# arghyasur1991/Spark-TTS

Measured on AMD Instinct MI355X. Metric: audio samples/sec (whole node), Spark-TTS-0.5B greedy, higher is better.
Workload: dtype bf16 weights + KV, fp32 activations/accumulate (LLM); vocoder: fp32 operands split into 2 bf16 planes, 3 products on the bf16 matrix pipe, fp32 accumulate

## Files before the change

spark-tts_amd/csrc/smi_llm.hip:

```cpp
#include "smi_common.h"
#include <stdio.h>
#include <string.h>
#include <cmath>
#include <map>
#include <mutex>
#include <vector>

namespace {

constexpr int kMaxRows = SMI_MAX_ROWS;
constexpr int kHeadDim = 64;

struct RowDesc {
  int32_t slot, pos, token, flags;
};

struct SampRec {
  int32_t mode;
  int32_t top_k;
  float inv_temp, top_p;
  unsigned long long seed;
  int32_t has_seed, pad;
};

// ... 1853 lines not shown
constexpr int kFuseOT = 2;

__device__ __forceinline__ void attn_merge(const float* wmax, const float (*pw)[kHeadDim], const float* pl, int d,
                                           float& bm, float& O, float& Ls) {
  constexpr float LOG2E = 1.4426950408889634f;
  float wm[kAttnWaves], po[kAttnWaves], pls[kAttnWaves];
#pragma unroll
  for (int w = 0; w < kAttnWaves; ++w) { wm[w] = wmax[w]; po[w] = pw[w][d]; pls[w] = pl[w]; }
  bm = wm[0];
#pragma unroll
  for (int w = 1; w < kAttnWaves; ++w) bm = fmaxf(bm, wm[w]);
  O = 0.f; Ls = 0.f;
#pragma unroll
  for (int w = 0; w < kAttnWaves; ++w) {
    const float sc = exp2f((wm[w] - bm) * LOG2E);
    O += po[w] * sc; Ls += pls[w] * sc;
  }
}

__device__ __forceinline__ void attn_merge_split(const float* wmax, const float (*pw)[kHeadDim], const float* pl, int d,
                                                 uint32_t& hi, uint32_t& mi, uint32_t& lo) {
  float bm, O, Ls;
  attn_merge(wmax, pw, pl, d, bm, O, Ls);
  split3(O / Ls, hi, mi, lo);
}

__device__ __forceinline__ void attn_put_pieces(unsigned char* xs, int d, uint32_t hi, uint32_t mi, uint32_t lo) {
  unsigned char* q = xs + (size_t)((d >> 5) * 12 + ((d >> 3) & 3)) * 16 + (d & 7) * 2;
  *(uint16_t*)q = (uint16_t)hi;
  *(uint16_t*)(q + 64) = (uint16_t)mi;
  *(uint16_t*)(q + 128) = (uint16_t)lo;
}

template <int KVF32, int ONE = 0, int FUSE = 0, int PG = 0>
__global__ __launch_bounds__((FUSE ? 2 : 1) * kAttnWaves * 64) void k_attn(AttnP p) {
  static_assert(!FUSE || (FUSE == 1 && ONE == 1) || (FUSE == 2 && ONE == 2), "fused o_proj: one row (per-head partials for gate_up) or 2..8 rows (last-arriver head sum)");
  constexpr int LPT = KVF32 ? 16 : 8;
  constexpr int DPL = kHeadDim / LPT;
  constexpr int TPW = 64 / LPT;
  constexpr int NGRP = kAttnWaves * TPW;
  constexpr int UNR = 4;
  constexpr float NEG = -1e30f;
  constexpr float LOG2E = 1.4426950408889634f;
  __shared__ float wmax[kAttnWaves];
  __shared__ __attribute__((aligned(16))) float so[kAttnWaves][TPW][kHeadDim];
  __shared__ float sl[kAttnWaves][TPW];
  __shared__ float pw[kAttnWaves][kHeadDim], pl[kAttnWaves];
  __shared__ __attribute__((aligned(16))) unsigned char xsl[FUSE == 1 ? kAttnWaves * 2 * 3 * 4 * 16 : FUSE ? 2 * 3 * 4 * 16 : 16];
  __shared__ unsigned int s_last;
  const int tid = threadIdx.x, lane = tid & 63, wave = tid >> 6;
  if constexpr (ONE == 1) {
    if constexpr (FUSE) asm volatile("" ::"s"(p.q), "s"(p.work_blocks), "s"(p.Wo), "s"(gridDim.x));
    else asm volatile("" ::"s"(p.q), "s"(p.work_blocks), "s"(gridDim.x));
  }
  if ((int)blockIdx.x >= p.work_blocks) {
    pf_run(p.pf, (int)blockIdx.x - p.work_blocks, (int)gridDim.x - p.work_blocks, tid, (FUSE ? 2 : 1) * kAttnWaves * 64);
    return;
  }
  unsigned fbid = blockIdx.x;
  if constexpr (FUSE == 2) {
    const unsigned total = (unsigned)p.work_blocks, xcd = fbid & 7u, slot = fbid >> 3, q8 = total >> 3, r8 = total & 7u;
    fbid = xcd * q8 + (xcd < r8 ? xcd : r8) + slot;
  }
  const int f_head = FUSE ? (int)(fbid % (unsigned)p.n_heads) : 0, f_q = FUSE ? (int)(fbid / (unsigned)p.n_heads) % kFuseQB : 0,
            f_row = FUSE == 2 ? (int)(fbid / (unsigned)(p.n_heads * kFuseQB)) : 0;
  if constexpr (FUSE) {
    if (wave >= kAttnWaves) {
      const int fq = f_q, fper = p.NTo / kFuseQB, fh = f_head;
      const int ow = wave - kAttnWaves, KTo = 2 * p.n_heads;
// ... 41 lines not shown
          }
        }
      }
      if constexpr (FUSE != 2) return;
      else asm volatile("s_waitcnt vmcnt(0)" ::: "memory");
    }
  }
  if (!FUSE || wave < kAttnWaves) {
  unsigned bid = blockIdx.x;
  if (ONE != 1) {
    const unsigned total = (unsigned)p.work_blocks, xcd = bid & 7u, slot = bid >> 3, q8 = total >> 3, r8 = total & 7u;
    bid = xcd * q8 + (xcd < r8 ? xcd : r8) + slot;
  }
  const int head = FUSE == 2 ? f_head : ONE == 1 ? (FUSE ? (int)bid % p.n_heads : (int)bid) : ONE == 2 ? (int)bid % p.n_heads : (int)(bid / p.nseg) % p.n_heads,
            m = FUSE == 2 ? f_row : ONE == 1 ? 0 : ONE == 2 ? (int)bid / p.n_heads : (int)bid / (p.nseg * p.n_heads),
            seg = ONE ? 0 : (int)bid % p.nseg;
  const int tl = lane / LPT, dl = lane % LPT;
  const int grp = wave * TPW + tl;
  const RowDesc rd = p.rows[m];
  const int kvh = head / p.group;
  const bool sir = ONE || p.slot_is_row;
  const int slot = sir ? m : rd.slot;
  const size_t rowbase = ((size_t)slot * p.n_kv + kvh) * p.max_pos;
  const int ctx_all = rd.pos + 1;
  int ctx = ctx_all < (seg + 1) * kAttnSeg ? ctx_all : (seg + 1) * kAttnSeg;
  if (!ONE && seg * kAttnSeg >= ctx_all) return;

  float qraw[DPL];
  {
    const float* qp = p.q + (size_t)m * p.q_dim + head * kHeadDim + dl * DPL;
#pragma unroll
    for (int i = 0; i < DPL; ++i) qraw[i] = qp[i];
  }
  float m_run = NEG, lrun = 0.f, o[DPL];
#pragma unroll
  for (int i = 0; i < DPL; ++i) o[i] = 0.f;

  int c0 = seg * kAttnSeg;
  do {
    uint4 kr[UNR], vr[UNR];
#pragma unroll
    for (int u = 0; u < UNR; ++u) {
      const int t = c0 + u * NGRP + grp;
      const int tc = sir ? (t < p.max_pos ? t : p.max_pos - 1) : (t < ctx ? t : ctx - 1);
      const size_t off = ((ONE && !PG) ? rowbase + tc : kv_row(p.km, slot, kvh, p.n_kv, p.max_pos, tc)) * kHeadDim + dl * DPL;
      if (KVF32) {
        kr[u] = *(const uint4*)((const float*)p.kcache + off);
        vr[u] = *(const uint4*)((const float*)p.vcache + off);
      } else {
        kr[u] = *(const uint4*)((const uint16_t*)p.kcache + off);
        vr[u] = *(const uint4*)((const uint16_t*)p.vcache + off);
      }
    }
    if (ONE) {
      int pr = rd.pos;
      asm volatile("" : "+v"(pr));
      ctx = pr + 1 < kAttnSeg ? pr + 1 : kAttnSeg;
    }
    float qv[DPL];
#pragma unroll
    for (int i = 0; i < DPL; ++i) {
      float t = qraw[i];
      asm volatile("" : "+v"(t));
      qv[i] = t * 0.125f;
    }
    float sc[UNR];
    float lmax = NEG;
#pragma unroll
    for (int u = 0; u < UNR; ++u) {
      const uint32_t ku[4] = {kr[u].x, kr[u].y, kr[u].z, kr[u].w};
      float d = 0.f;
      if (KVF32) {
#pragma unroll
        for (int i = 0; i < 4; ++i) d += qv[i % DPL] * __uint_as_float(ku[i]);
      } else {
#pragma unroll
        for (int i = 0; i < 4; ++i) {
          d += qv[(2 * i) % DPL] * __uint_as_float(ku[i] << 16);
          d += qv[(2 * i + 1) % DPL] * __uint_as_float(ku[i] & 0xffff0000u);
        }
      }
      d = KVF32 ? smi_sum16(d) : smi_sum8(d);
      sc[u] = (c0 + u * NGRP + grp < ctx) ? d : NEG;
      lmax = fmaxf(lmax, sc[u]);
    }
    lmax = fmaxf(lmax, smi_dpp<0x128>(lmax));
    const float wm = fmaxf(fmaxf(smi_readlane(lmax, 0), smi_readlane(lmax, 16)), fmaxf(smi_readlane(lmax, 32), smi_readlane(lmax, 48)));
    const float mn = fmaxf(m_run, wm);
    const float a = exp2f((m_run - mn) * LOG2E);
    lrun *= a;
#pragma unroll
    for (int i = 0; i < DPL; ++i) o[i] *= a;
#pragma unroll
    for (int u = 0; u < UNR; ++u) {
      const float e = sc[u] > 0.5f * NEG ? exp2f((sc[u] - mn) * LOG2E) : 0.f;
      const uint32_t vu[4] = {vr[u].x, vr[u].y, vr[u].z, vr[u].w};
      lrun += e;
      if (KVF32) {
#pragma unroll
        for (int i = 0; i < 4; ++i) o[i % DPL] += e * __uint_as_float(vu[i]);
      } else {
#pragma unroll
        for (int i = 0; i < 4; ++i) {
          o[(2 * i) % DPL] += e * __uint_as_float(vu[i] << 16);
          o[(2 * i + 1) % DPL] += e * __uint_as_float(vu[i] & 0xffff0000u);
        }
      }
    }
    m_run = mn;
    c0 += NGRP * UNR;
  } while (c0 < ctx);
#pragma unroll
  for (int i = 0; i < DPL; i += 4)
    *(float4*)&so[wave][tl][dl * DPL + i] = make_float4(o[i], o[i + 1], o[i + 2], o[i + 3]);
  if (dl == 0) sl[wave][tl] = lrun;
  asm volatile("s_waitcnt lgkmcnt(0)" ::: "memory");
  {
    float O = 0.f, Ls = 0.f;
#pragma unroll
    for (int g = 0; g < TPW; ++g) { O += so[wave][g][lane]; Ls += sl[wave][g]; }
    pw[wave][lane] = O;
    if (lane == 0) { pl[wave] = Ls; wmax[wave] = m_run; }
  }
  __syncthreads();
  if constexpr (FUSE == 1) return;
  if (tid < kHeadDim) {
    if (!ONE && p.nseg > 1) {
      float bm, O, Ls;
      attn_merge(wmax, pw, pl, tid, bm, O, Ls);
      float* pp = p.part + (((size_t)m * p.n_heads + head) * p.nseg + seg) * 66;
      pp[2 + tid] = O;
      if (tid == 0) { pp[0] = bm; pp[1] = Ls; }
      return;
    }
    uint32_t hi, mi, lo;
    attn_merge_split(wmax, pw, pl, tid, hi, mi, lo);
    if constexpr (FUSE) {
      attn_put_pieces(xsl, tid, hi, mi, lo);
    } else {
      const int Mx = ONE == 1 ? 1 : p.M;
      const size_t ob = xs_off(o_ktile(head, tid, p.n_heads), 0, (tid >> 3) & 3, m, Mx) + (tid & 7) * 2;
      const size_t pl2 = (size_t)4 * Mx * 16;
      *(uint16_t*)(p.xs_out + ob) = (uint16_t)hi;
      *(uint16_t*)(p.xs_out + ob + pl2) = (uint16_t)mi;
// ... 1007 lines not shown
  int pg_split_rows;
  int pg_forced;
  float *part_o, *h2;
  float4* dpart;
  int dc_min;
  int fuse_o;
  int fuse1_last;
  int fuse2_rows;
  unsigned int* fuse_cnt;
  RowDesc* rows;
  RowDesc* plan;
  PfTile* pf_tiles;
  size_t pf_tiles_cap;
  int pf_ntiles;
  std::vector<PfTile> host_tiles;
  int attn_pf2;
  size_t plan_cap;
  float* pval; int* pidx; int lm_blocks, lm_cap;
  int64_t* hist; int32_t *count, *finished, *step;
  void *kcache, *vcache; size_t kv_layer_elems;
  int B; int started;
  int paged, pshift, ppslot;
  int32_t* ptab;
  std::vector<int32_t> hptab;
  std::vector<int32_t> free_pages;
  std::vector<int32_t> page_ref;
  int slot_pages[kMaxRows];
  int plen[kMaxRows];
  Ctl hctl; Ctl* ctl;
  int admit_seq;
  int session, identity_slots;
  std::vector<int> live_order;
  int attn_seg;
  float* apart; size_t apart_floats;
  int slot_busy[kMaxRows], slot_len[kMaxRows];
  int max_len, steps_launched;
  int do_sample, top_k; float temperature, top_p; unsigned long long seed;
  int slot_samp[kMaxRows];
  int slot_pen[kMaxRows];
  int slot_lp[kMaxRows];
  int slot_allow[kMaxRows];
  int lm_restrict;
  int* tlist;
  std::vector<int32_t> host_tlist;
  float* lp;
  float* lp_part; float2* lp_rowc;
  uint16_t* phist;
  int64_t* poll_dev; int64_t* poll_host;
  int32_t* pen_idx; size_t pen_idx_cap;
  std::vector<int32_t> host_pen_idx;
  float* logits; int* tok;
  float* cand_v; int* cand_i; unsigned int* cand_n;
  unsigned long long* stamps; int stamps_on;
  int max_steps;
  int tune[4];
  int graph_steps;
  int pf_inline;
  int pf_qkv_eighths;
  int prefetch_mask, prefetch_rows;
  int tune2;
  int pgemm_min_rows;
  int pg_min[4];
  int wd_parts;
  int exact;
  int gu1_lo;
  int gu1_rows;
  hipGraphExec_t graph; int graph_B, graph_seg, graph_ident, graph_samp, graph_pen, graph_lp, graph_allow;
  std::map<hipGraphExec_t, hipStream_t> graph_last;
  std::map<uint64_t, hipGraphExec_t> graph_cache;
  hipEvent_t ev0, ev1;
  std::vector<RowDesc> host_rows;
#ifdef SMI_DIAG
  EngState eng;
  int eng_on;
#endif
};

namespace {

std::vector<const void*>& lds_big_kernels() {
  static std::vector<const void*> v;
  return v;
}
bool lds_big_register(const void* f) {
  lds_big_kernels().push_back(f);
  return true;
}
template <auto F>
struct LdsBig {
  static inline const bool reg = lds_big_register((const void*)F);
};
constexpr int kLdsBigBytes = 160 * 1024;

void pages_release(smi_llm* L, int slot) {
  for (int i = 0; i < L->slot_pages[slot]; ++i) {
    const int32_t pg = L->hptab[(size_t)slot * L->ppslot + i];
    if (--L->page_ref[pg] == 0) L->free_pages.push_back(pg);
  }
  L->slot_pages[slot] = 0;
}
// ... 31 lines not shown
  return SMI_OK;
}
KvMap kv_map(const smi_llm* L) { return KvMap{L->paged ? L->ptab : nullptr, L->pshift, L->ppslot}; }
bool samp_any(const smi_llm* L) {
  if (L->do_sample) return true;
  for (int sl = 0; sl < kMaxRows; ++sl)
    if (L->slot_samp[sl]) return true;
  return false;
}
bool pen_any(const smi_llm* L) {
  for (int sl = 0; sl < kMaxRows; ++sl)
    if (L->slot_pen[sl]) return true;
  return false;
}
bool lp_any(const smi_llm* L) {
  for (int sl = 0; sl < kMaxRows; ++sl)
    if (L->slot_lp[sl]) return true;
  return false;
}
bool allow_any(const smi_llm* L) {
  for (int sl = 0; sl < kMaxRows; ++sl)
    if (L->slot_allow[sl]) return true;
  return false;
}
bool lm_restricted(const smi_llm* L) {
  return L->lm_restrict && L->KTh <= 32 && !L->exact && allow_any(L);
}
bool logits_needed(const smi_llm* L) {
  return samp_any(L) || pen_any(L) || lp_any(L) || (allow_any(L) && !lm_restricted(L));
}
int allow_bits(const smi_llm* L) { return allow_any(L) ? (lm_restricted(L) ? 3 : 1) : 0; }
uint64_t graph_key(const smi_llm* L, int samp, int pen, int lp, int K) {
  return (uint64_t)L->B | ((uint64_t)L->attn_seg << 8) | ((uint64_t)(L->identity_slots ? 1 : 0) << 24) | ((uint64_t)samp << 25) |
         ((uint64_t)pen << 26) | ((uint64_t)lp << 27) | ((uint64_t)allow_bits(L) << 28) | ((uint64_t)K << 32);
}
void graphs_flush(smi_llm* L) {
  std::vector<hipStream_t> drained;
  for (auto& gl : L->graph_last) {
    bool seen = false;
    for (hipStream_t d : drained) seen |= d == gl.second;
    if (!seen) { (void)hipStreamSynchronize(gl.second); drained.push_back(gl.second); }
  }
  L->graph_last.clear();
  for (auto& kv : L->graph_cache) if (kv.second) (void)hipGraphExecDestroy(kv.second);
  L->graph_cache.clear();
  L->graph = nullptr;
}

template <int MT, int NTB, int NW, int U, int WB, int PRO, int EPI, int H = 1, int OCC = 1>
int launch_gemm_kv(const smi_llm* L, GemmP p, hipStream_t st) {
  const int work = (p.NT + NTB - 1) / NTB * H;
  p.work_blocks = work;
  p.stamps = L->stamps_on ? L->stamps : nullptr;
  if constexpr (MT == 1 && NTB == 1 && NW == 16 && H == 4 && PRO == PRO_PLAIN && EPI == EPI_RESID) {
    if (p.M == 1 && !p.stamps && p.KT <= 160 && !(L->tune2 & 1048576)) {
      const int helpers = (L->prefetch_mask & 4) && p.pf.base && work < 232 ? ((L->tune2 & 4194304) ? 224 : (256 - work) / 8 * 8) : 0;
      if (p.KT <= 32) hipLaunchKernelGGL(k_down1<2>, dim3(work + helpers), dim3(256), 0, st, p);
      else if (p.KT <= 96) hipLaunchKernelGGL(k_down1<6>, dim3(work + helpers), dim3(256), 0, st, p);
      else hipLaunchKernelGGL(k_down1<10>, dim3(work + helpers), dim3(256), 0, st, p);
      SMI_LAUNCH_CHECK();
      return SMI_OK;
    }
    if (p.M >= 2 && p.M <= 8 && !p.stamps && p.KT <= 160 && !(L->tune2 & 2097152)) {
      const dim3 g(work), b(256);
      if (p.M <= 4) {
        if (p.KT <= 32) hipLaunchKernelGGL((k_downS<2, 1>), g, b, 0, st, p);
        else if (p.KT <= 96) hipLaunchKernelGGL((k_downS<6, 1>), g, b, 0, st, p);
// ... 222 lines not shown

enum { KQKV = 0, KATTN, KO, KGU, KD, KLM, KFIN };
enum { PF_GROUPED = 1, PF_PGEMM = 2 };
constexpr int kPgSplitRows = 512;
constexpr int kPgSegO = 2, kPgSegD = 8;

int ensure_apart(smi_llm* L, size_t floats) {
  if (floats <= L->apart_floats) return SMI_OK;
  graphs_flush(L);
  if (L->apart) (void)hipFree(L->apart);
  L->apart = nullptr; L->apart_floats = 0;
  if (hipMalloc((void**)&L->apart, floats * 4) != hipSuccess) { smi_set_error("hipMalloc(attention partials, %zu floats) failed", floats); return SMI_ENOMEM; }
  L->apart_floats = floats;
  return SMI_OK;
}

int lm_blocks_for(const smi_llm* L, int M) {
  if (L->KTh > 32 || L->exact) return L->lm_cap;
  return M <= 16 ? L->lm_blocks : (L->lm_blocks < 256 ? L->lm_blocks : 256);
}

int pen_set_ids(int V, int nblk) { return ((V + nblk - 1) / nblk + 3) & ~3; }

LpP lp_params(const smi_llm* L, int M) {
  LpP lp;
  lp.logits = L->logits; lp.ctl = L->ctl; lp.rows = L->rows; lp.pval = L->pval; lp.nblk = lm_blocks_for(L, M);
  lp.V = L->cfg.vocab_size; lp.per = pen_set_ids(lp.V, kLpBlocks); lp.inv_temp = 1.0f / L->temperature; lp.hs = L->do_sample;
  lp.part = L->lp_part; lp.rowc = L->lp_rowc;
  return lp;
}

int segs_for(int ctx_bound) { return ctx_bound <= kAttnSeg ? 1 : (ctx_bound + kAttnSeg - 1) / kAttnSeg; }

template <int KVF32>
int launch_attn(smi_llm* L, AttnP a, int helpers_ok, hipStream_t st) {
  a.nseg = L->attn_seg < 1 ? 1 : L->attn_seg;
  a.work_blocks = a.n_heads * a.M * a.nseg;
  const bool fuse = a.M == 1 && a.nseg == 1 && a.slot_is_row && a.part_o && !a.cnt;
  const bool fuse2 = a.nseg == 1 && a.slot_is_row && a.part_o && a.cnt;
  if (fuse || fuse2) a.work_blocks *= kFuseQB;
  if (a.nseg > 1) {
    int rc = ensure_apart(L, (size_t)a.M * a.n_heads * a.nseg * 66);
    if (rc) return rc;
    a.part = L->apart;
  }
  const int helpers = (helpers_ok && (L->prefetch_mask & 2) && a.M <= L->prefetch_rows && a.work_blocks < 232) ? (256 - a.work_blocks) / 8 * 8 : 0;
  const bool pg = a.km.ptab != nullptr;
#ifdef SMI_DIAG
  if (fuse2 && pg)
    hipLaunchKernelGGL((k_attn<KVF32, 2, 2, 1>), dim3(a.work_blocks), dim3(2 * kAttnWaves * 64), 0, st, a);
  else if (fuse2)
    hipLaunchKernelGGL((k_attn<KVF32, 2, 2>), dim3(a.work_blocks), dim3(2 * kAttnWaves * 64), 0, st, a);
  else
#endif
  if (fuse && pg)
    hipLaunchKernelGGL((k_attn<KVF32, 1, 1, 1>), dim3(a.work_blocks + helpers), dim3(2 * kAttnWaves * 64), 0, st, a);
  else if (fuse)
    hipLaunchKernelGGL((k_attn<KVF32, 1, 1>), dim3(a.work_blocks + helpers), dim3(2 * kAttnWaves * 64), 0, st, a);
  else if (a.M == 1 && a.nseg == 1 && a.slot_is_row && pg)
    hipLaunchKernelGGL((k_attn<KVF32, 1, 0, 1>), dim3(a.work_blocks + helpers), dim3(kAttnWaves * 64), 0, st, a);
  else if (a.M == 1 && a.nseg == 1 && a.slot_is_row)
    hipLaunchKernelGGL((k_attn<KVF32, 1>), dim3(a.work_blocks + helpers), dim3(kAttnWaves * 64), 0, st, a);
  else if (a.nseg == 1 && a.slot_is_row && pg)
    hipLaunchKernelGGL((k_attn<KVF32, 2, 0, 1>), dim3(a.work_blocks + helpers), dim3(kAttnWaves * 64), 0, st, a);
  else if (a.nseg == 1 && a.slot_is_row)
    hipLaunchKernelGGL((k_attn<KVF32, 2>), dim3(a.work_blocks + helpers), dim3(kAttnWaves * 64), 0, st, a);
  else
    hipLaunchKernelGGL((k_attn<KVF32, 0>), dim3(a.work_blocks + helpers), dim3(kAttnWaves * 64), 0, st, a);
  SMI_LAUNCH_CHECK();
  if (a.nseg > 1) {
    hipLaunchKernelGGL(k_attn_merge, dim3(a.M), dim3(1024), 0, st, a);
    SMI_LAUNCH_CHECK();
  }
  return SMI_OK;
}

bool fuse_o_now(const smi_llm* L, const RowDesc* rows, int M) {
  return L->fuse_o && !L->fuse1_last && M == 1 && rows == L->rows && L->identity_slots && L->attn_seg <= 1;
}
bool fuse2_now(const smi_llm* L, const RowDesc* rows, int M) {
  return L->fuse_o && M >= (L->fuse1_last ? 1 : 2) && M <= L->fuse2_rows && rows == L->rows && L->identity_slots && L->attn_seg <= 1;
}

int launch_oproj(const smi_llm* L, const GemmP& p, int M, hipStream_t st) {
  switch (L->cfg.num_heads) {
    case 14: return M <= 8 ? launch_gemm<1, 14, 2, 1, PRO_PLAIN, EPI_RESID, 4>(L, p, st) : launch_gemm<1, 14, 2, 1, PRO_PLAIN, EPI_RESID, 1, 0>(L, p, st);
    case 4: return M <= 8 ? launch_gemm<1, 4, 2, 1, PRO_PLAIN, EPI_RESID, 4>(L, p, st) : launch_gemm<1, 4, 2, 1, PRO_PLAIN, EPI_RESID, 1, 0>(L, p, st);
    default:
      return M <= 8 ? launch_gemm<1, 8, 4, 1, PRO_PLAIN, EPI_RESID, 4>(L, p, st) : launch_gemm<1, 8, 4, 1, PRO_PLAIN, EPI_RESID, 1, 0>(L, p, st);
  }
}

template <int TPC, int MTN>
int launch_down_chains_t(const smi_llm* L, const DownCP& d, hipStream_t st) {
  const size_t lds = (size_t)TPC * 12 * (d.M < MTN * 16 ? d.M : MTN * 16) * 16;
  static_cast<void>(LdsBig<k_downC<TPC, MTN>>::reg);
// ... 487 lines not shown
  { L->tune[0] = L->tune[1] = L->tune[2] = L->tune[3] = 0; const char* e = smi_env("SPARKMI_TUNE"); if (e) sscanf(e, "%d,%d,%d,%d", &L->tune[0], &L->tune[1], &L->tune[2], &L->tune[3]); }
  L->bh = L->bq = nullptr; L->bxs_h = L->bxs_attn = L->bxs_act = nullptr; L->bss = nullptr; L->big_rows = 0;
  L->pslab = nullptr; L->pslab_bytes = 0;
  L->prefetch_mask = 1; L->prefetch_rows = 1;
  if (const char* e = smi_env("SPARKMI_PREFETCH")) { L->prefetch_mask = atoi(e) & 7; L->prefetch_rows = 8; }
  if (smi_env("SPARKMI_NO_PREFETCH")) L->prefetch_mask = 0;
  { const char* e = smi_env("SPARKMI_GRAPH_STEPS"); L->graph_steps = e ? atoi(e) : 8; if (L->graph_steps < 1 || L->graph_steps > 32) L->graph_steps = 8; }
  { const char* e = smi_env("SPARKMI_PF_INLINE"); L->pf_inline = !(e && e[0] == '0'); }
  { const char* e = smi_env("SPARKMI_PF_QKV"); L->pf_qkv_eighths = e ? atoi(e) : 2; if (L->pf_qkv_eighths < 0 || L->pf_qkv_eighths > 8) L->pf_qkv_eighths = 2; }
  L->part_o = nullptr; L->h2 = nullptr; L->dpart = nullptr; L->fuse_cnt = nullptr;
  { const char* e = smi_env("SPARKMI_FUSE1_LAST"); L->fuse1_last = e && e[0] == '1'; }
  { const char* e = smi_env("SPARKMI_FUSE2_ROWS"); L->fuse2_rows = e ? atoi(e) : 0; if (L->fuse2_rows > kFuse2Max) L->fuse2_rows = kFuse2Max; }
  { const char* e = smi_env("SPARKMI_DC_MIN"); L->dc_min = e ? atoi(e) : 7; }
  L->fuse_o = !smi_env("SPARKMI_NO_FUSE_O") && (cfg->num_heads == 14 || cfg->num_heads == 4) && cfg->num_heads <= kMaxOHeads &&
              L->NTh % kFuseQB == 0 && L->NTh / kFuseQB <= kAttnWaves * kFuseOT && L->KTh * 8 <= 256;
  { const char* e = smi_env("SPARKMI_TUNE2"); L->tune2 = e ? atoi(e) : 0; }
  { const char* e = smi_env("SPARKMI_PGEMM_MIN_ROWS"); L->pgemm_min_rows = e ? atoi(e) : 1280; }
  {
    const char* names[4] = {"SPARKMI_PGEMM_MIN_QKV", "SPARKMI_PGEMM_MIN_O", "SPARKMI_PGEMM_MIN_GU", "SPARKMI_PGEMM_MIN_D"};
    const int dflt[4] = {1280, 1280, 288, 896};
    const bool common = smi_env("SPARKMI_PGEMM_MIN_ROWS") != nullptr;
    L->pg_forced = common;
    for (int i = 0; i < 4; ++i) { const char* e = smi_env(names[i]); L->pg_forced |= e != nullptr; L->pg_min[i] = e ? atoi(e) : common ? L->pgemm_min_rows : dflt[i]; }
  }
  { const char* e = smi_env("SPARKMI_PG_SPLIT_ROWS"); L->pg_split_rows = e ? atoi(e) : kPgSplitRows; if (L->pg_split_rows > kPgSplitRows) L->pg_split_rows = kPgSplitRows; }
  { const char* e = smi_env("SPARKMI_PF_LONG"); L->pf_long = e ? atoi(e) : kMaxRows + 1; if (L->pf_long < kMaxRows + 1) L->pf_long = kMaxRows + 1; }
  { const char* e = smi_env("SPARKMI_GU1_ROWS"); L->gu1_rows = e ? atoi(e) : 32; }
  { const char* e = smi_env("SPARKMI_GU1_LO"); L->gu1_lo = e ? atoi(e) : 4; }
  L->wd_parts = cfg->wd_plain ? 0 : 1;
  L->exact = cfg->weights_exact;
  if (L->exact) L->fuse_o = 0;
  L->pf_tiles = nullptr; L->pf_tiles_cap = 0; L->pf_ntiles = 0;
  { const char* e = smi_env("SPARKMI_ATTN_PF2"); L->attn_pf2 = !(e && e[0] == '0'); }
  L->graph = nullptr; L->graph_B = 0; L->graph_seg = 1; L->graph_ident = 1; L->graph_samp = 0; L->graph_pen = 0; L->graph_lp = 0; L->graph_allow = 0; memset(L->slot_samp, 0, sizeof(L->slot_samp)); memset(L->slot_pen, 0, sizeof(L->slot_pen));
  memset(L->slot_lp, 0, sizeof(L->slot_lp)); L->lp = nullptr; L->lp_part = nullptr; L->lp_rowc = nullptr;
  memset(L->slot_allow, 0, sizeof(L->slot_allow)); L->lm_restrict = 0; L->tlist = nullptr;
  L->poll_dev = nullptr; L->poll_host = nullptr;
  L->phist = nullptr; L->pen_idx = nullptr; L->pen_idx_cap = 0; L->plan = nullptr; L->plan_cap = 0; L->B = 0; L->started = 0; L->ctl = nullptr; L->admit_seq = 0; memset(&L->hctl, 0, sizeof(L->hctl));
  L->session = 0; L->identity_slots = 1; L->attn_seg = 1; L->apart = nullptr; L->apart_floats = 0; memset(L->slot_busy, 0, sizeof(L->slot_busy)); memset(L->slot_len, 0, sizeof(L->slot_len));
  const size_t esz = cfg->kv_dtype ? 4 : 2;
  L->paged = cfg->kv_page_tokens > 0; L->pshift = 0; L->ppslot = 0; L->ptab = nullptr;
  memset(L->slot_pages, 0, sizeof(L->slot_pages)); memset(L->plen, 0, sizeof(L->plen));
  L->kv_layer_elems = (size_t)cfg->max_slots * cfg->num_kv_heads * cfg->max_positions * kHeadDim;
  if (L->paged) {
    while ((1 << L->pshift) < cfg->kv_page_tokens) ++L->pshift;
    L->ppslot = cfg->max_positions >> L->pshift;
    L->kv_layer_elems = (size_t)cfg->kv_pages * cfg->num_kv_heads * cfg->kv_page_tokens * kHeadDim;
    L->hptab.assign((size_t)cfg->max_slots * L->ppslot, 0);
    for (int pg = cfg->kv_pages - 1; pg >= 0; --pg) L->free_pages.push_back(pg);
    L->page_ref.assign((size_t)cfg->kv_pages, 0);
  }
  const size_t kvbytes = L->kv_layer_elems * esz * cfg->num_layers;
#define SMI_ALLOC(ptr, bytes)                                                      \
  if (hipMalloc((void**)&(ptr), (bytes)) != hipSuccess) {                          \
    smi_set_error("hipMalloc(%s, %zu bytes) failed", #ptr, (size_t)(bytes));       \
    smi_llm_destroy(L);                                                            \
    return SMI_ENOMEM;                                                             \
  }
  SMI_ALLOC(L->h, (size_t)kMaxRows * L->H * 4);
  SMI_ALLOC(L->qbuf, (size_t)kMaxRows * L->Q * 4);
  SMI_ALLOC(L->xs_h, (size_t)kMaxRows * L->H * 6);
  SMI_ALLOC(L->xs_attn, (size_t)kMaxRows * L->Q * 6);
  SMI_ALLOC(L->xs_act, (size_t)kMaxRows * L->I * 6);
  SMI_ALLOC(L->sspart, (size_t)kMaxRows * L->NTh * 4 * 4);
  SMI_ALLOC(L->part_o, (size_t)kFuse2Max * kMaxOHeads * L->H * 4);
  SMI_ALLOC(L->fuse_cnt, (size_t)kFuse2Max * kFuseQB * 4);
  SMI_HIP(hipMemset(L->fuse_cnt, 0, (size_t)kFuse2Max * kFuseQB * 4));
  SMI_ALLOC(L->h2, (size_t)L->H * 4);
  SMI_ALLOC(L->dpart, (size_t)16 * L->NTh * 4 * 64 * 16);
  SMI_ALLOC(L->rows, kMaxRows * sizeof(RowDesc));
  SMI_ALLOC(L->pval, (size_t)L->lm_cap * kMaxRows * 4);
  SMI_ALLOC(L->pidx, (size_t)L->lm_cap * kMaxRows * 4);
// ... 768 lines not shown
      smi_set_error("smi_llm_slots_logprobs: the sequence in slot %d was admitted without return_log_probs", slots[i]);
      return SMI_ESTATE;
    }
  hipStream_t st = (hipStream_t)stream;
  int32_t cnt[kMaxRows];
  SMI_HIP(hipMemcpyAsync(cnt, L->count, kMaxRows * 4, hipMemcpyDeviceToHost, st));
  int steps = cap < L->max_steps ? cap : L->max_steps;
  std::vector<float> lp((size_t)steps * kMaxRows);
  SMI_HIP(hipMemcpyAsync(lp.data(), L->lp, lp.size() * 4, hipMemcpyDeviceToHost, st));
  SMI_HIP(hipStreamSynchronize(st));
  for (int i = 0; i < n; ++i) {
    int k = cnt[slots[i]] < steps ? cnt[slots[i]] : steps;
    for (int t = 0; t < k; ++t) out_host[(size_t)i * cap + t] = lp[(size_t)t * kMaxRows + slots[i]];
    n_out[i] = k;
  }
  return SMI_OK;
}

int smi_llm_slot_tokens(smi_llm* L, int slot, int64_t* out, int cap, int32_t* n_out, int32_t* finished, void* stream) {
  SMI_REQUIRE(L && out && n_out && finished && slot >= 0 && slot < kMaxRows && cap >= 0, "smi_llm_slot_tokens: bad argument");
  hipStream_t st = (hipStream_t)stream;
  int32_t cnt = 0, fin = 0;
  SMI_HIP(hipMemcpyAsync(&cnt, L->count + slot, 4, hipMemcpyDeviceToHost, st));
  SMI_HIP(hipMemcpyAsync(&fin, L->finished + slot, 4, hipMemcpyDeviceToHost, st));
  SMI_HIP(hipStreamSynchronize(st));
  int n = cnt < cap ? cnt : cap;
  if (n > L->max_steps) n = L->max_steps;
  if (n > 0) SMI_HIP(hipMemcpy2D(out, 8, L->hist + slot, kMaxRows * 8, 8, (size_t)n, hipMemcpyDeviceToHost));
  *n_out = n;
  *finished = fin;
  return SMI_OK;
}

int smi_llm_decode(smi_llm* L, int n_steps, void* stream) {
  SMI_REQUIRE(L, "smi_llm_decode: null handle");
  if (!L->started) { smi_set_error("smi_llm_decode before smi_llm_prefill"); return SMI_ESTATE; }
  SMI_REQUIRE(n_steps >= 0, "smi_llm_decode: n_steps < 0");
  if (L->session) {
    if (L->B == 0 || n_steps == 0) return SMI_OK;
    for (int sl = 0; sl < kMaxRows; ++sl)
      if (L->slot_busy[sl])
        SMI_REQUIRE(L->slot_len[sl] + n_steps <= L->cfg.max_positions, "smi_llm_decode: %d more steps would take slot %d past max_positions=%d",
                    n_steps, sl, L->cfg.max_positions);
  } else {
    SMI_REQUIRE(L->max_len + L->steps_launched + n_steps <= L->cfg.max_positions,
                "smi_llm_decode: %d more steps would pass max_positions=%d (prompt %d, %d steps so far)", n_steps,
                L->cfg.max_positions, L->max_len, L->steps_launched);
  }
  hipStream_t st = (hipStream_t)stream;
  int rc;
  if (L->paged && n_steps > 0) {
    int sl[kMaxRows], need[kMaxRows], n = 0;
    if (L->session) {
      for (int s2 = 0; s2 < kMaxRows; ++s2)
        if (L->slot_busy[s2]) { sl[n] = s2; need[n++] = L->slot_len[s2] + n_steps; }
    } else {
      for (int b = 0; b < L->B; ++b) { sl[n] = b; need[n++] = L->plen[b] + L->steps_launched + n_steps; }
    }
    for (int i = 0; i < n; ++i) need[i] = need[i] < L->cfg.max_positions ? need[i] : L->cfg.max_positions;
    if ((rc = pages_ensure(L, sl, need, n, st))) return rc;
  }
  {
    int bound = L->max_len + L->steps_launched + n_steps;
    if (L->session) {
      bound = 0;
      for (int sl = 0; sl < kMaxRows; ++sl)
        if (L->slot_busy[sl] && L->slot_len[sl] + n_steps > bound) bound = L->slot_len[sl] + n_steps;
    }
    L->attn_seg = segs_for(bound);
    if (L->attn_seg > 1 && (rc = ensure_apart(L, (size_t)kMaxRows * L->cfg.num_heads * L->attn_seg * 66))) return rc;
  }
  const int samp = samp_any(L) ? 1 : 0, pen = pen_any(L) ? 1 : 0, lpb = lp_any(L) ? 1 : 0, alw = allow_bits(L);
  if (L->cfg.use_graph && n_steps > 0 && (!L->graph || L->graph_B != L->B || L->graph_seg != L->attn_seg || L->graph_ident != L->identity_slots ||
                                          L->graph_samp != samp || L->graph_pen != pen || L->graph_lp != lpb || L->graph_allow != alw)) {
    const uint64_t key = graph_key(L, samp, pen, lpb, 0);
    auto hit = L->graph_cache.find(key);
    L->graph = hit != L->graph_cache.end() ? hit->second : nullptr;
    L->graph_B = L->B; L->graph_seg = L->attn_seg; L->graph_ident = L->identity_slots; L->graph_samp = samp; L->graph_pen = pen; L->graph_lp = lpb; L->graph_allow = alw;
  }
  if (L->cfg.use_graph && n_steps > 0 && !L->graph) {
    const uint64_t key = graph_key(L, samp, pen, lpb, 0);
    if (L->graph_cache.size() >= 192) graphs_flush(L);
    hipStream_t cs;
    SMI_HIP(hipStreamCreateWithFlags(&cs, hipStreamNonBlocking));
    hipGraph_t g = nullptr;
    hipError_t e = hipStreamBeginCapture(cs, hipStreamCaptureModeThreadLocal);
    if (e == hipSuccess) {
      rc = launch_step(L, L->B, cs);
      hipError_t e2 = hipStreamEndCapture(cs, &g);
      if (rc == SMI_OK && e2 == hipSuccess && g) {
        if (hipGraphInstantiate(&L->graph, g, nullptr, nullptr, 0) != hipSuccess) L->graph = nullptr;
      }
      if (g) (void)hipGraphDestroy(g);
    }
    (void)hipStreamDestroy(cs);
    (void)hipGetLastError();
    L->graph_B = L->B; L->graph_seg = L->attn_seg; L->graph_ident = L->identity_slots; L->graph_samp = samp; L->graph_pen = pen; L->graph_lp = lpb; L->graph_allow = alw;
    if (!L->graph) { smi_set_error("hipGraph capture of the decode step failed"); return SMI_EHIP; }
    L->graph_cache[key] = L->graph;
  }
  int s0 = 0;
  if (L->cfg.use_graph && L->graph_steps > 1 && n_steps >= L->graph_steps) {
    const int K = L->graph_steps;
    const uint64_t keyk = graph_key(L, samp, pen, lpb, K);
    hipGraphExec_t gk = nullptr;
    auto hit = L->graph_cache.find(keyk);
    if (hit != L->graph_cache.end()) gk = hit->second;
    else if (n_steps >= 2 * K && L->graph_cache.size() < 192) {
      hipStream_t cs;
      SMI_HIP(hipStreamCreateWithFlags(&cs, hipStreamNonBlocking));
      hipGraph_t g = nullptr;
      hipError_t e = hipStreamBeginCapture(cs, hipStreamCaptureModeThreadLocal);
      if (e == hipSuccess) {
        rc = SMI_OK;
        for (int k = 0; k < K && rc == SMI_OK; ++k) rc = launch_step(L, L->B, cs);
        hipError_t e2 = hipStreamEndCapture(cs, &g);
        if (rc == SMI_OK && e2 == hipSuccess && g && hipGraphInstantiate(&gk, g, nullptr, nullptr, 0) != hipSuccess) gk = nullptr;
        if (g) (void)hipGraphDestroy(g);
      }
      (void)hipStreamDestroy(cs);
      (void)hipGetLastError();
      if (gk) L->graph_cache[keyk] = gk;
    }
    if (gk) {
      for (; s0 + K <= n_steps; s0 += K) {
        SMI_HIP(hipGraphLaunch(gk, st));
        L->graph_last[gk] = st;
      }
    }
  }
// ... 112 lines not shown
    for (int k = KQKV; k < kernel && rc == SMI_OK; ++k) rc = launch_one(L, k, layer, L->rows, L->B, nullptr, 0);
    if (rc) return rc;
  }
  L->stamps_on = 1;
  rc = launch_one(L, kernel, layer, L->rows, L->B, nullptr, 0);
  L->stamps_on = 0;
  if (rc) return rc;
  SMI_HIP(hipDeviceSynchronize());
  std::vector<unsigned long long> h((size_t)4096 * 8);
  SMI_HIP(hipMemcpy(h.data(), L->stamps, h.size() * 8, hipMemcpyDeviceToHost));
  int nblk = 0;
  while (nblk < 4096 && h[(size_t)nblk * 8]) ++nblk;
  SMI_REQUIRE(nblk > 0, "smi_llm_debug_stamps: the kernel left no stamps");
  unsigned long long t0 = ~0ull;
  for (int b = 0; b < nblk; ++b) t0 = h[(size_t)b * 8] < t0 ? h[(size_t)b * 8] : t0;
  for (int i = 0; i < 7; ++i) {
    double s = 0;
    for (int b = 0; b < nblk; ++b) s += (double)(h[(size_t)b * 8 + i] - t0);
    out[i] = s / nblk * 0.01;
  }
  double cyc = 0, us = 0;
  for (int b = 0; b < nblk; ++b) { cyc += (double)h[(size_t)b * 8 + 7]; us += (double)(h[(size_t)b * 8 + 6] - h[(size_t)b * 8]) * 0.01; }
  out[7] = us > 0 ? cyc / us : 0;
  return SMI_OK;
}

int smi_llm_time_kernel(smi_llm* L, int kernel, int layer, int iters, float* ms_avg, void* stream) {
  SMI_REQUIRE(L && ms_avg && iters > 0, "smi_llm_time_kernel: bad argument");
  SMI_REQUIRE((kernel >= 0 && kernel <= 8) || (kernel >= 16 && kernel <= 16 + KD), "smi_llm_time_kernel: kernel id %d", kernel);
  if (!L->started) { smi_set_error("smi_llm_time_kernel needs a started generation (prefill first)"); return SMI_ESTATE; }
  if (L->paged && kernel != 7) { smi_set_error("smi_llm_time_kernel: the per-kernel probes need a contiguous KV cache (kv_page_tokens = 0)"); return SMI_ESTATE; }
  hipStream_t st = (hipStream_t)stream;
  int rc;
  if (kernel == 8) {
    const bool eng = eng_usable(L, L->rows, L->B);
    if ((rc = eng ? eng_launch(L, st) : launch_layers(L, L->rows, L->B, false, st))) return rc;
    SMI_HIP(hipEventRecord(L->ev0, st));
    for (int i = 0; i < iters; ++i)
      if ((rc = eng ? eng_launch(L, st) : launch_layers(L, L->rows, L->B, false, st))) return rc;
    SMI_HIP(hipEventRecord(L->ev1, st));
    L->started = 0;
  } else if (kernel == 7) {
    if ((rc = smi_llm_decode(L, 1, stream))) return rc;
    SMI_HIP(hipEventRecord(L->ev0, st));
    if ((rc = smi_llm_decode(L, iters, stream))) return rc;
    SMI_HIP(hipEventRecord(L->ev1, st));
  } else if (kernel >= 16) {
    const int k = kernel - 16, nl = L->cfg.num_layers;
    SMI_REQUIRE(k >= KQKV && k <= KD, "smi_llm_time_kernel: in-sequence timing is for the layer kernels");
    float t[2] = {0.f, 0.f};
    for (int pass = 0; pass < 2; ++pass) {
      hipStream_t cs;
      SMI_HIP(hipStreamCreateWithFlags(&cs, hipStreamNonBlocking));
      hipGraph_t g = nullptr;
      hipGraphExec_t ge = nullptr;
      rc = SMI_OK;
      hipError_t e = hipStreamBeginCapture(cs, hipStreamCaptureModeThreadLocal);
      if (e == hipSuccess) {
        for (int i = 0; i < iters && rc == SMI_OK; ++i) {
          const int l = (layer + i) % nl;
          for (int kk = KQKV; kk <= KD && rc == SMI_OK; ++kk)
            if (!(pass == 1 && kk == k)) rc = launch_one(L, kk, l, L->rows, L->B, nullptr, cs);
        }
        e = hipStreamEndCapture(cs, &g);
      }
      if (e == hipSuccess && rc == SMI_OK && g) e = hipGraphInstantiate(&ge, g, nullptr, nullptr, 0);
// ... 174 lines not shown
      const unsigned char* base = (const unsigned char*)kv_layer(L, isv ? L->vcache : L->kcache, layer);
      const size_t row0 = ((size_t)slot * nkv + kh) * L->cfg.max_positions + pos0;
      SMI_HIP(hipMemcpy(buf.data(), base + row0 * kHeadDim * esz, buf.size(), hipMemcpyDeviceToHost));
      for (int t = 0; t < n; ++t)
        for (int i = 0; i < kHeadDim; ++i) {
          const int d = isv ? i : (i >> 1) + 32 * (i & 1);
          float x;
          if (f32) x = ((const float*)buf.data())[(size_t)t * kHeadDim + i];
          else { const uint32_t u = (uint32_t)((const uint16_t*)buf.data())[(size_t)t * kHeadDim + i] << 16; memcpy(&x, &u, 4); }
          (isv ? v_host : k_host)[((size_t)t * nkv + kh) * kHeadDim + d] = x;
        }
    }
  return SMI_OK;
}

int smi_llm_debug_layer(smi_llm* L, int layer, int M, const int32_t* rows_host, const float* hidden_host, int stage) {
  SMI_REQUIRE(L && rows_host && hidden_host && M >= 1 && M <= kMaxRows, "smi_llm_debug_layer: bad argument");
  SMI_REQUIRE(layer >= 0 && layer < L->cfg.num_layers && stage >= 0 && stage <= 4, "smi_llm_debug_layer: layer %d stage %d", layer, stage);
  SMI_REQUIRE(!L->paged, "smi_llm_debug_layer needs a contiguous KV cache");
  SMI_HIP(hipDeviceSynchronize());
  graphs_flush(L);
  std::vector<RowDesc> rows(kMaxRows, RowDesc{0, 0, 0, 0});
  int maxpos = 0, ident = 1;
  for (int m = 0; m < M; ++m) {
    const int sl = rows_host[2 * m], ps = rows_host[2 * m + 1];
    SMI_REQUIRE(sl >= 0 && sl < L->cfg.max_slots && ps >= 0 && ps < L->cfg.max_positions, "smi_llm_debug_layer: row %d = (slot %d, pos %d)", m, sl, ps);
    rows[m] = RowDesc{sl, ps, 0, 0};
    maxpos = ps > maxpos ? ps : maxpos;
    ident &= sl == m;
  }
  SMI_HIP(hipMemcpy(L->rows, rows.data(), rows.size() * sizeof(RowDesc), hipMemcpyHostToDevice));
  L->B = M; L->identity_slots = ident; L->session = 0; L->started = 0;
  L->attn_seg = segs_for(maxpos + 1);
  float* src = nullptr;
  SMI_HIP(hipMalloc((void**)&src, (size_t)M * L->H * 4));
  int rc = SMI_OK;
  if (hipMemcpy(src, hidden_host, (size_t)M * L->H * 4, hipMemcpyHostToDevice) != hipSuccess) { rc = SMI_EHIP; smi_set_error("smi_llm_debug_layer: upload failed"); }
  if (rc == SMI_OK) {
    hipLaunchKernelGGL(k_load_hidden, dim3((M + 3) / 4), dim3(256), 0, 0, src, L->KTh, M, (const float*)sec(L, SMI_LLM_LN1, layer), L->h, L->xs_h,
                       L->sspart, L->NTh * 4);
    if (hipGetLastError() != hipSuccess) { rc = SMI_EHIP; smi_set_error("smi_llm_debug_layer: k_load_hidden launch failed"); }
  }
  const bool fused = fuse_o_now(L, L->rows, M);
  const int last = (fused && stage == 2) ? KGU : KQKV + stage;
  for (int k = KQKV; k <= last && rc == SMI_OK; ++k) rc = launch_one(L, k, layer, L->rows, M, nullptr, 0);
  if (hipDeviceSynchronize() != hipSuccess && rc == SMI_OK) { rc = SMI_EHIP; smi_set_error("smi_llm_debug_layer: kernels failed: %s", hipGetErrorString(hipGetLastError())); }
  (void)hipFree(src);
  return rc;
}

int smi_llm_debug_raw_stamps(smi_llm* L, unsigned long long* out, int n) {
  SMI_REQUIRE(L && out && n > 0 && n <= 4096 * 8, "smi_llm_debug_raw_stamps: bad argument");
  SMI_HIP(hipDeviceSynchronize());
  SMI_HIP(hipMemcpy(out, L->stamps, (size_t)n * 8, hipMemcpyDeviceToHost));
  return SMI_OK;
}

int smi_llm_debug_sample(smi_llm* L, const float* logits_host, int n_rows, uint64_t seed, int use_bound, int32_t* tokens_out) {
  SMI_REQUIRE(L && tokens_out && n_rows >= 1 && n_rows <= kMaxRows, "smi_llm_debug_sample: bad argument");
  SMI_REQUIRE(L->do_sample, "smi_llm_debug_sample: smi_llm_set_sampling(do_sample = 1, ...) first");
  const int V = L->cfg.vocab_size;
  const int nblk = lm_blocks_for(L, n_rows);
  SMI_HIP(hipDeviceSynchronize());
  if (logits_host) {
    for (int m = 0; m < kMaxRows; ++m) SMI_HIP(hipMemcpy(L->logits + (size_t)m * V, logits_host, (size_t)V * 4, hipMemcpyHostToDevice));
    std::vector<float> pv((size_t)kMaxRows * L->lm_cap, -INFINITY);
    const int per = (V + nblk - 1) / nblk;
    for (int j = 0; j < nblk; ++j) {
      float mx = -INFINITY;
      for (int i = j * per; i < V && i < (j + 1) * per; ++i) mx = logits_host[i] > mx ? logits_host[i] : mx;
      for (int m = 0; m < kMaxRows; ++m) pv[(size_t)m * nblk + j] = mx;
    }
    SMI_HIP(hipMemcpy(L->pval, pv.data(), (size_t)kMaxRows * nblk * 4, hipMemcpyHostToDevice));
  }
  std::vector<RowDesc> rows(kMaxRows, RowDesc{0, 0, 0, 0});
  for (int m = 0; m < kMaxRows; ++m) { rows[m].slot = m; L->hctl.seqid[m] = m; }
  memset(L->hctl.samp, 0, sizeof(L->hctl.samp));
  memset(L->hctl.pen, 0, sizeof(L->hctl.pen));
  L->hctl.seed = seed;
  SMI_HIP(hipMemcpy(L->rows, rows.data(), rows.size() * sizeof(RowDesc), hipMemcpyHostToDevice));
// ... 148 lines not shown
```

Before: 567,300.

## Specialize single-row decode attention on host-chosen KV chunk count, splitting decode runs

Adds an NCH template parameter to the one-row attention kernel so that, when the context fits in one (or optionally two) unrolled chunks, the KV loads are issued up front as straight-line code with no loop. The intent is to issue all KV loads before the context-length check and the math, removing loop overhead and load-use serialization. The host splits decode runs at chunk boundaries so each graph is captured with the right chunk count, and the chunk count is added to the graph cache key. This adds more kernel instantiations and more graph captures, and extra graph switches around the boundary for batch-one decode.

```diff
diff --git a/spark-tts_amd/csrc/smi_llm.hip b/spark-tts_amd/csrc/smi_llm.hip
--- a/spark-tts_amd/csrc/smi_llm.hip
+++ b/spark-tts_amd/csrc/smi_llm.hip
@@ -1909,9 +1909,10 @@
   *(uint16_t*)(q + 128) = (uint16_t)lo;
 }
 
-template <int KVF32, int ONE = 0, int FUSE = 0, int PG = 0>
+template <int KVF32, int ONE = 0, int FUSE = 0, int PG = 0, int NCH = 0>
 __global__ __launch_bounds__((FUSE ? 2 : 1) * kAttnWaves * 64) void k_attn(AttnP p) {
   static_assert(!FUSE || (FUSE == 1 && ONE == 1) || (FUSE == 2 && ONE == 2), "fused o_proj: one row (per-head partials for gate_up) or 2..8 rows (last-arriver head sum)");
+  static_assert(NCH == 0 || (ONE == 1 && NCH <= 2), "a host-chosen chunk count: the one-row kernel, one or two chunks");
   constexpr int LPT = KVF32 ? 16 : 8;
   constexpr int DPL = kHeadDim / LPT;
   constexpr int TPW = 64 / LPT;
@@ -2019,13 +2020,12 @@
 #pragma unroll
     for (int i = 0; i < DPL; ++i) qraw[i] = qp[i];
   }
+  if constexpr (NCH != 0) asm volatile("" ::: "memory");
   float m_run = NEG, lrun = 0.f, o[DPL];
 #pragma unroll
   for (int i = 0; i < DPL; ++i) o[i] = 0.f;
 
-  int c0 = seg * kAttnSeg;
-  do {
-    uint4 kr[UNR], vr[UNR];
+  auto load_chunk = [&](int c0, uint4 (&kr)[UNR], uint4 (&vr)[UNR]) {
 #pragma unroll
     for (int u = 0; u < UNR; ++u) {
       const int t = c0 + u * NGRP + grp;
@@ -2039,11 +2039,13 @@
         vr[u] = *(const uint4*)((const uint16_t*)p.vcache + off);
       }
     }
-    if (ONE) {
-      int pr = rd.pos;
-      asm volatile("" : "+v"(pr));
-      ctx = pr + 1 < kAttnSeg ? pr + 1 : kAttnSeg;
-    }
+  };
+  auto late_ctx = [&]() {
+    int pr = rd.pos;
+    asm volatile("" : "+v"(pr));
+    ctx = pr + 1 < kAttnSeg ? pr + 1 : kAttnSeg;
+  };
+  auto chunk_math = [&](int c0, const uint4 (&kr)[UNR], const uint4 (&vr)[UNR]) {
     float qv[DPL];
 #pragma unroll
     for (int i = 0; i < DPL; ++i) {
@@ -2095,8 +2097,41 @@
       }
     }
     m_run = mn;
-    c0 += NGRP * UNR;
-  } while (c0 < ctx);
+  };
+  auto landed = [&](uint4 (&kr)[UNR], uint4 (&vr)[UNR]) {
+#pragma unroll
+    for (int u = 0; u < UNR; ++u) {
+      typedef uint32_t u32x4 __attribute__((ext_vector_type(4)));
+      u32x4 k4 = __builtin_bit_cast(u32x4, kr[u]), v4 = __builtin_bit_cast(u32x4, vr[u]);
+      asm volatile("" : "+v"(k4), "+v"(v4)::"memory");
+      kr[u] = __builtin_bit_cast(uint4, k4); vr[u] = __builtin_bit_cast(uint4, v4);
+    }
+  };
+  if constexpr (NCH == 1) {
+    uint4 kr[UNR], vr[UNR];
+    load_chunk(0, kr, vr);
+    landed(kr, vr);
+    late_ctx();
+    chunk_math(0, kr, vr);
+  } else if constexpr (NCH == 2) {
+    uint4 kr0[UNR], vr0[UNR], kr1[UNR], vr1[UNR];
+    load_chunk(0, kr0, vr0);
+    load_chunk(NGRP * UNR, kr1, vr1);
+    landed(kr0, vr0);
+    late_ctx();
+    chunk_math(0, kr0, vr0);
+    landed(kr1, vr1);
+    if (NGRP * UNR < ctx) chunk_math(NGRP * UNR, kr1, vr1);
+  } else {
+    int c0 = seg * kAttnSeg;
+    do {
+      uint4 kr[UNR], vr[UNR];
+      load_chunk(c0, kr, vr);
+      if (ONE) late_ctx();
+      chunk_math(c0, kr, vr);
+      c0 += NGRP * UNR;
+    } while (c0 < ctx);
+  }
 #pragma unroll
   for (int i = 0; i < DPL; i += 4)
     *(float4*)&so[wave][tl][dl * DPL + i] = make_float4(o[i], o[i + 1], o[i + 2], o[i + 3]);
@@ -3170,6 +3205,9 @@
   int session, identity_slots;
   std::vector<int> live_order;
   int attn_seg;
+  int attn_nch;
+  int attn_loop;
+  int attn_nch2;
   float* apart; size_t apart_floats;
   int slot_busy[kMaxRows], slot_len[kMaxRows];
   int max_len, steps_launched;
@@ -3203,7 +3241,7 @@
   int exact;
   int gu1_lo;
   int gu1_rows;
-  hipGraphExec_t graph; int graph_B, graph_seg, graph_ident, graph_samp, graph_pen, graph_lp, graph_allow;
+  hipGraphExec_t graph; int graph_B, graph_seg, graph_nch, graph_ident, graph_samp, graph_pen, graph_lp, graph_allow;
   std::map<hipGraphExec_t, hipStream_t> graph_last;
   std::map<uint64_t, hipGraphExec_t> graph_cache;
   hipEvent_t ev0, ev1;
@@ -3301,7 +3339,7 @@
 int allow_bits(const smi_llm* L) { return allow_any(L) ? (lm_restricted(L) ? 3 : 1) : 0; }
 uint64_t graph_key(const smi_llm* L, int samp, int pen, int lp, int K) {
   return (uint64_t)L->B | ((uint64_t)L->attn_seg << 8) | ((uint64_t)(L->identity_slots ? 1 : 0) << 24) | ((uint64_t)samp << 25) |
-         ((uint64_t)pen << 26) | ((uint64_t)lp << 27) | ((uint64_t)allow_bits(L) << 28) | ((uint64_t)K << 32);
+         ((uint64_t)pen << 26) | ((uint64_t)lp << 27) | ((uint64_t)allow_bits(L) << 28) | ((uint64_t)(L->attn_nch & 3) << 30) | ((uint64_t)K << 32);
 }
 void graphs_flush(smi_llm* L) {
   std::vector<hipStream_t> drained;
@@ -3590,6 +3628,13 @@
 
 int segs_for(int ctx_bound) { return ctx_bound <= kAttnSeg ? 1 : (ctx_bound + kAttnSeg - 1) / kAttnSeg; }
 
+int attn_chunk(const smi_llm* L) { return L->cfg.kv_dtype ? 128 : 256; }
+int attn_nch_for(const smi_llm* L, int ctx_bound) {
+  if (L->attn_loop) return 0;
+  const int ch = attn_chunk(L);
+  return ctx_bound <= ch ? 1 : (L->attn_nch2 && ctx_bound <= 2 * ch) ? 2 : 0;
+}
+
 template <int KVF32>
 int launch_attn(smi_llm* L, AttnP a, int helpers_ok, hipStream_t st) {
   a.nseg = L->attn_seg < 1 ? 1 : L->attn_seg;
@@ -3611,15 +3656,26 @@
     hipLaunchKernelGGL((k_attn<KVF32, 2, 2>), dim3(a.work_blocks), dim3(2 * kAttnWaves * 64), 0, st, a);
   else
 #endif
-  if (fuse && pg)
-    hipLaunchKernelGGL((k_attn<KVF32, 1, 1, 1>), dim3(a.work_blocks + helpers), dim3(2 * kAttnWaves * 64), 0, st, a);
-  else if (fuse)
-    hipLaunchKernelGGL((k_attn<KVF32, 1, 1>), dim3(a.work_blocks + helpers), dim3(2 * kAttnWaves * 64), 0, st, a);
-  else if (a.M == 1 && a.nseg == 1 && a.slot_is_row && pg)
-    hipLaunchKernelGGL((k_attn<KVF32, 1, 0, 1>), dim3(a.work_blocks + helpers), dim3(kAttnWaves * 64), 0, st, a);
-  else if (a.M == 1 && a.nseg == 1 && a.slot_is_row)
-    hipLaunchKernelGGL((k_attn<KVF32, 1>), dim3(a.work_blocks + helpers), dim3(kAttnWaves * 64), 0, st, a);
-  else if (a.nseg == 1 && a.slot_is_row && pg)
+  if (a.M == 1 && a.nseg == 1 && a.slot_is_row) {
+    const dim3 g1(a.work_blocks + helpers);
+    switch ((fuse ? 2 : 0) + (pg ? 1 : 0) + 4 * L->attn_nch) {
+      case 0: hipLaunchKernelGGL((k_attn<KVF32, 1, 0, 0, 0>), g1, dim3(kAttnWaves * 64), 0, st, a); break;
+      case 1: hipLaunchKernelGGL((k_attn<KVF32, 1, 0, 1, 0>), g1, dim3(kAttnWaves * 64), 0, st, a); break;
+      case 2: hipLaunchKernelGGL((k_attn<KVF32, 1, 1, 0, 0>), g1, dim3(2 * kAttnWaves * 64), 0, st, a); break;
+      case 3: hipLaunchKernelGGL((k_attn<KVF32, 1, 1, 1, 0>), g1, dim3(2 * kAttnWaves * 64), 0, st, a); break;
+      case 4: hipLaunchKernelGGL((k_attn<KVF32, 1, 0, 0, 1>), g1, dim3(kAttnWaves * 64), 0, st, a); break;
+      case 5: hipLaunchKernelGGL((k_attn<KVF32, 1, 0, 1, 1>), g1, dim3(kAttnWaves * 64), 0, st, a); break;
+      case 6: hipLaunchKernelGGL((k_attn<KVF32, 1, 1, 0, 1>), g1, dim3(2 * kAttnWaves * 64), 0, st, a); break;
+      case 7: hipLaunchKernelGGL((k_attn<KVF32, 1, 1, 1, 1>), g1, dim3(2 * kAttnWaves * 64), 0, st, a); break;
+#ifdef SMI_DIAG
+      case 8: hipLaunchKernelGGL((k_attn<KVF32, 1, 0, 0, 2>), g1, dim3(kAttnWaves * 64), 0, st, a); break;
+      case 9: hipLaunchKernelGGL((k_attn<KVF32, 1, 0, 1, 2>), g1, dim3(kAttnWaves * 64), 0, st, a); break;
+      case 10: hipLaunchKernelGGL((k_attn<KVF32, 1, 1, 0, 2>), g1, dim3(2 * kAttnWaves * 64), 0, st, a); break;
+      case 11: hipLaunchKernelGGL((k_attn<KVF32, 1, 1, 1, 2>), g1, dim3(2 * kAttnWaves * 64), 0, st, a); break;
+#endif
+      default: smi_set_error("launch_attn: chunk count %d", L->attn_nch); return SMI_EINVAL;
+    }
+  } else if (a.nseg == 1 && a.slot_is_row && pg)
     hipLaunchKernelGGL((k_attn<KVF32, 2, 0, 1>), dim3(a.work_blocks + helpers), dim3(kAttnWaves * 64), 0, st, a);
   else if (a.nseg == 1 && a.slot_is_row)
     hipLaunchKernelGGL((k_attn<KVF32, 2>), dim3(a.work_blocks + helpers), dim3(kAttnWaves * 64), 0, st, a);
@@ -4173,12 +4229,12 @@
   if (L->exact) L->fuse_o = 0;
   L->pf_tiles = nullptr; L->pf_tiles_cap = 0; L->pf_ntiles = 0;
   { const char* e = smi_env("SPARKMI_ATTN_PF2"); L->attn_pf2 = !(e && e[0] == '0'); }
-  L->graph = nullptr; L->graph_B = 0; L->graph_seg = 1; L->graph_ident = 1; L->graph_samp = 0; L->graph_pen = 0; L->graph_lp = 0; L->graph_allow = 0; memset(L->slot_samp, 0, sizeof(L->slot_samp)); memset(L->slot_pen, 0, sizeof(L->slot_pen));
+  L->graph = nullptr; L->graph_B = 0; L->graph_seg = 1; L->graph_nch = 0; L->graph_ident = 1; L->graph_samp = 0; L->graph_pen = 0; L->graph_lp = 0; L->graph_allow = 0; memset(L->slot_samp, 0, sizeof(L->slot_samp)); memset(L->slot_pen, 0, sizeof(L->slot_pen));
   memset(L->slot_lp, 0, sizeof(L->slot_lp)); L->lp = nullptr; L->lp_part = nullptr; L->lp_rowc = nullptr;
   memset(L->slot_allow, 0, sizeof(L->slot_allow)); L->lm_restrict = 0; L->tlist = nullptr;
   L->poll_dev = nullptr; L->poll_host = nullptr;
   L->phist = nullptr; L->pen_idx = nullptr; L->pen_idx_cap = 0; L->plan = nullptr; L->plan_cap = 0; L->B = 0; L->started = 0; L->ctl = nullptr; L->admit_seq = 0; memset(&L->hctl, 0, sizeof(L->hctl));
-  L->session = 0; L->identity_slots = 1; L->attn_seg = 1; L->apart = nullptr; L->apart_floats = 0; memset(L->slot_busy, 0, sizeof(L->slot_busy)); memset(L->slot_len, 0, sizeof(L->slot_len));
+  L->session = 0; L->identity_slots = 1; L->attn_seg = 1; L->attn_nch = 0; L->attn_loop = smi_env("SPARKMI_ATTN_LOOP") != nullptr; L->attn_nch2 = smi_env("SPARKMI_ATTN_NCH2") != nullptr; L->apart = nullptr; L->apart_floats = 0; memset(L->slot_busy, 0, sizeof(L->slot_busy)); memset(L->slot_len, 0, sizeof(L->slot_len));
   const size_t esz = cfg->kv_dtype ? 4 : 2;
   L->paged = cfg->kv_page_tokens > 0; L->pshift = 0; L->ppslot = 0; L->ptab = nullptr;
   memset(L->slot_pages, 0, sizeof(L->slot_pages)); memset(L->plen, 0, sizeof(L->plen));
@@ -5013,6 +5069,9 @@
   return SMI_OK;
 }
 
+static int decode_ctx_bound(const smi_llm* L, int n_steps);
+static int decode_unit(smi_llm* L, int n_steps, void* stream);
+
 int smi_llm_decode(smi_llm* L, int n_steps, void* stream) {
   SMI_REQUIRE(L, "smi_llm_decode: null handle");
   if (!L->started) { smi_set_error("smi_llm_decode before smi_llm_prefill"); return SMI_ESTATE; }
@@ -5029,7 +5088,7 @@
                 L->cfg.max_positions, L->max_len, L->steps_launched);
   }
   hipStream_t st = (hipStream_t)stream;
-  int rc;
+  int rc = SMI_OK;
   if (L->paged && n_steps > 0) {
     int sl[kMaxRows], need[kMaxRows], n = 0;
     if (L->session) {
@@ -5041,23 +5100,46 @@
     for (int i = 0; i < n; ++i) need[i] = need[i] < L->cfg.max_positions ? need[i] : L->cfg.max_positions;
     if ((rc = pages_ensure(L, sl, need, n, st))) return rc;
   }
+  if (L->B == 1 && L->identity_slots && !L->attn_loop && n_steps > 0) {
+    const int ch = attn_chunk(L);
+    while (n_steps > 0 && rc == SMI_OK) {
+      const int cur = decode_ctx_bound(L, 0);
+      const int n = cur < ch ? ch - cur : (L->attn_nch2 && cur < 2 * ch) ? 2 * ch - cur : n_steps;
+      const int part = n < n_steps ? n : n_steps;
+      rc = decode_unit(L, part, stream);
+      n_steps -= part;
+    }
+  } else {
+    rc = decode_unit(L, n_steps, stream);
+  }
+  L->attn_nch = 0;
+  return rc;
+}
+
+static int decode_ctx_bound(const smi_llm* L, int n_steps) {
+  if (!L->session) return L->max_len + L->steps_launched + n_steps;
+  int bound = 0;
+  for (int sl = 0; sl < kMaxRows; ++sl)
+    if (L->slot_busy[sl] && L->slot_len[sl] + n_steps > bound) bound = L->slot_len[sl] + n_steps;
+  return bound;
+}
+
+static int decode_unit(smi_llm* L, int n_steps, void* stream) {
+  hipStream_t st = (hipStream_t)stream;
+  int rc;
   {
-    int bound = L->max_len + L->steps_launched + n_steps;
-    if (L->session) {
-      bound = 0;
-      for (int sl = 0; sl < kMaxRows; ++sl)
-        if (L->slot_busy[sl] && L->slot_len[sl] + n_steps > bound) bound = L->slot_len[sl] + n_steps;
-    }
+    const int bound = decode_ctx_bound(L, n_steps);
     L->attn_seg = segs_for(bound);
+    L->attn_nch = L->B == 1 && L->identity_slots ? attn_nch_for(L, bound) : 0;
     if (L->attn_seg > 1 && (rc = ensure_apart(L, (size_t)kMaxRows * L->cfg.num_heads * L->attn_seg * 66))) return rc;
   }
   const int samp = samp_any(L) ? 1 : 0, pen = pen_any(L) ? 1 : 0, lpb = lp_any(L) ? 1 : 0, alw = allow_bits(L);
-  if (L->cfg.use_graph && n_steps > 0 && (!L->graph || L->graph_B != L->B || L->graph_seg != L->attn_seg || L->graph_ident != L->identity_slots ||
+  if (L->cfg.use_graph && n_steps > 0 && (!L->graph || L->graph_B != L->B || L->graph_seg != L->attn_seg || L->graph_nch != L->attn_nch || L->graph_ident != L->identity_slots ||
                                           L->graph_samp != samp || L->graph_pen != pen || L->graph_lp != lpb || L->graph_allow != alw)) {
     const uint64_t key = graph_key(L, samp, pen, lpb, 0);
     auto hit = L->graph_cache.find(key);
     L->graph = hit != L->graph_cache.end() ? hit->second : nullptr;
-    L->graph_B = L->B; L->graph_seg = L->attn_seg; L->graph_ident = L->identity_slots; L->graph_samp = samp; L->graph_pen = pen; L->graph_lp = lpb; L->graph_allow = alw;
+    L->graph_B = L->B; L->graph_seg = L->attn_seg; L->graph_nch = L->attn_nch; L->graph_ident = L->identity_slots; L->graph_samp = samp; L->graph_pen = pen; L->graph_lp = lpb; L->graph_allow = alw;
   }
   if (L->cfg.use_graph && n_steps > 0 && !L->graph) {
     const uint64_t key = graph_key(L, samp, pen, lpb, 0);
@@ -5076,7 +5158,7 @@
     }
     (void)hipStreamDestroy(cs);
     (void)hipGetLastError();
-    L->graph_B = L->B; L->graph_seg = L->attn_seg; L->graph_ident = L->identity_slots; L->graph_samp = samp; L->graph_pen = pen; L->graph_lp = lpb; L->graph_allow = alw;
+    L->graph_B = L->B; L->graph_seg = L->attn_seg; L->graph_nch = L->attn_nch; L->graph_ident = L->identity_slots; L->graph_samp = samp; L->graph_pen = pen; L->graph_lp = lpb; L->graph_allow = alw;
     if (!L->graph) { smi_set_error("hipGraph capture of the decode step failed"); return SMI_EHIP; }
     L->graph_cache[key] = L->graph;
   }
@@ -5255,6 +5337,8 @@
   if (L->paged && kernel != 7) { smi_set_error("smi_llm_time_kernel: the per-kernel probes need a contiguous KV cache (kv_page_tokens = 0)"); return SMI_ESTATE; }
   hipStream_t st = (hipStream_t)stream;
   int rc;
+  struct NchScope { smi_llm* L; ~NchScope() { L->attn_nch = 0; } } nch_scope{L};
+  if (kernel != 7) L->attn_nch = L->B == 1 && L->identity_slots ? attn_nch_for(L, decode_ctx_bound(L, 1)) : 0;
   if (kernel == 8) {
     const bool eng = eng_usable(L, L->rows, L->B);
     if ((rc = eng ? eng_launch(L, st) : launch_layers(L, L->rows, L->B, false, st))) return rc;
@@ -5495,6 +5579,7 @@
   SMI_HIP(hipMemcpy(L->rows, rows.data(), rows.size() * sizeof(RowDesc), hipMemcpyHostToDevice));
   L->B = M; L->identity_slots = ident; L->session = 0; L->started = 0;
   L->attn_seg = segs_for(maxpos + 1);
+  L->attn_nch = M == 1 && ident ? attn_nch_for(L, maxpos + 1) : 0;
   float* src = nullptr;
   SMI_HIP(hipMalloc((void**)&src, (size_t)M * L->H * 4));
   int rc = SMI_OK;
@@ -5509,6 +5594,7 @@
   for (int k = KQKV; k <= last && rc == SMI_OK; ++k) rc = launch_one(L, k, layer, L->rows, M, nullptr, 0);
   if (hipDeviceSynchronize() != hipSuccess && rc == SMI_OK) { rc = SMI_EHIP; smi_set_error("smi_llm_debug_layer: kernels failed: %s", hipGetErrorString(hipGetLastError())); }
   (void)hipFree(src);
+  L->attn_nch = 0;
   return rc;
 }
 
```

Result: no change. 567,700, median of 2 (+0.1%).
